# lalitkrajendran/photon

Measured on AMD Instinct MI355X. Metric: Mrays/sec, 1e7-ray 256^3 BOS render, higher is better.
Workload: dtype f32

## Files before the change

### photon_amd/csrc/device_volume_coop.hpp

```cpp
#pragma once
#include "../../include/photon_philox.h"
#include "device_volume.hpp"

namespace photon {

enum PathSlot : int {
    PS_C_COHERENT,
    PS_C_HIT_CELL,
    PS_C_CELL_IN_TILE,
    PS_C_FETCH_UP,
    PS_C_FETCH_DOWN,
    PS_C_TILE_CLAMPED,
    PS_C_INCOHERENT,
    PS_C_INCOHERENT_LANES,
    PS_C_BRICK_PASS,
    PS_C_BRICK_FETCH,
    PS_C_BRICK_REUSED,
    PS_C_BRICK_CLAMPED,
    PS_C_BRICK_LANES,
    PS_C_GATHER_LANES,
    PS_C_SPIN_OUTSIDE,
    PS_C_SPIN_LOW,
    PS_C_SPIN_CAP,
    PS_L_COHERENT,
    PS_L_HIT_A,
    PS_L_HIT_B,
    PS_L_TILE_B_LANES,
    PS_L_FETCH,
    PS_L_FETCH_TWO,
    PS_L_FETCH_TO_B,
    PS_L_FETCH_DOWN,
    PS_L_BASE_AHEAD,
    PS_L_BASE_BEHIND,
    PS_L_TILE_CLAMPED,
    PS_L_NO_FREE_TILE,
    PS_L_OUT_OF_REACH,
    PS_L_MARK_INCOHERENT,
    PS_L_TILES_SKIPPED,
    PS_L_RETRY,
    PS_L_COHERENT_AGAIN,
    PS_L_INCOHERENT,
    PS_L_INCOHERENT_LANES,
    PS_L_BRICK_PASS,
    PS_L_BRICK_FETCH,
    PS_L_BRICK_REUSED,
    PS_L_BRICK_CLAMPED,
    PS_L_BRICK_LANES,
    PS_L_GATHER_LANES,
    PS_L_SPIN_OUTSIDE,
    PS_L_SPIN_CAP,
    PS_L_LOW,
    PS_L_REPAIR_LANES,
    PS_L_KEEP_PREV_LANES,
    PS_COUNT
};
constexpr int kPathSlots = PS_COUNT;
#ifndef PHOTON_PATH_STATS
#define PHOTON_PATH_STATS 0
#endif
#if PHOTON_PATH_STATS
__device__ unsigned long long g_path_stats[kPathSlots];
__device__ __forceinline__ void path_stat(PathSlot k, unsigned long long n = 1) {
    if ((int)(threadIdx.x & 63) == __ffsll((long long)ballot(true)) - 1) atomicAdd(&g_path_stats[k], n);
}
__device__ __forceinline__ void path_stat_if(PathSlot k, bool c) { if (c) path_stat(k); }
__device__ __forceinline__ void path_lanes(PathSlot k, unsigned long long mask) { if (mask != 0) path_stat(k, (unsigned long long)__popcll(mask)); }
#else
#define path_stat(...) ((void)0)
#define path_stat_if(...) ((void)0)
#define path_lanes(...) ((void)0)
#endif

#ifndef PHOTON_BRICK_PASSES
#define PHOTON_BRICK_PASSES 6
#endif
#ifndef PHOTON_LINEAR_TILE_LAYERS
#define PHOTON_LINEAR_TILE_LAYERS 16
#endif
#ifndef PHOTON_LINEAR_TILES
#define PHOTON_LINEAR_TILES 2
#endif
#ifndef PHOTON_TILE_RETRY_MASK
#define PHOTON_TILE_RETRY_MASK 15
#endif
#ifndef PHOTON_BRICK_PITCH
#define PHOTON_BRICK_PITCH 12
#endif
constexpr int kBrickPitch = PHOTON_BRICK_PITCH;
constexpr int kBrickSlab = 8 * kBrickPitch;
#ifndef PHOTON_CUBIC_TILE_LAYERS
#define PHOTON_CUBIC_TILE_LAYERS 7
#endif
constexpr int kCubicTileLayers = PHOTON_CUBIC_TILE_LAYERS;
static_assert(kCubicTileLayers >= 4 && kCubicTileLayers <= 8, "PHOTON_CUBIC_TILE_LAYERS");
template <int INTERP> constexpr int tile_texels() { return INTERP == 2 ? 16 * kCubicTileLayers : PHOTON_LINEAR_TILES * PHOTON_LINEAR_TILE_LAYERS * 4; }
#ifndef PHOTON_SPINS_IN_LDS
#define PHOTON_SPINS_IN_LDS 1
#endif
constexpr int kSpinSlotTexels = PHOTON_SPINS_IN_LDS ? 32 : 0;
template <int INTERP> constexpr int wave_lds_texels() { return tile_texels<INTERP>() + (INTERP == 2 ? 4 : 2) * kBrickSlab + (INTERP == 1 ? kSpinSlotTexels : 0); }
constexpr int kWaveLdsTexels = wave_lds_texels<2>();

template <int RS, int SS>
__device__ __forceinline__ f4 cubic_taps_lds(const f4 *blk, const float (&wx)[4], const float (&wy)[4],
                                             const float (&wz)[4]) {
    float wxy[4][4];
#pragma unroll
    for (int b = 0; b < 4; b++)
#pragma unroll
        for (int a = 0; a < 4; a++) wxy[b][a] = wx[a] * wy[b];
    f4 acc = f4{0, 0, 0, 0}, s = f4{0, 0, 0, 0};
    float w0 = wxy[0][0];
    f4 t[4];
#pragma unroll
    for (int a = 0; a < 4; a++) t[a] = ldtexel(blk + a);
#pragma unroll
    for (int r = 0; r < 16; r++) {
        const int b = r & 3, c = r >> 2;
#pragma unroll
        for (int a = 0; a < 4; a++) {
            const f4 ta = t[a];
            const float w = (a == 0 && b == 0) ? w0 : wxy[b][a];
            if (a == 0 && b == 0) s = f4{w * ta.x, w * ta.y, w * ta.z, w * ta.w};
            else s = f4{fmaf(w, ta.x, s.x), fmaf(w, ta.y, s.y), fmaf(w, ta.z, s.z), fmaf(w, ta.w, s.w)};
            asm volatile("" : "+v"(s.x), "+v"(s.y), "+v"(s.z), "+v"(s.w) : : "memory");
            if (r < 15) t[a] = ldtexel(blk + ((r + 1) >> 2) * SS + ((r + 1) & 3) * RS + a);
            asm volatile("" : "+v"(w0) : : "memory");
        }
        if (b == 3) {
            if (c == 0) acc = f4{wz[0] * s.x, wz[0] * s.y, wz[0] * s.z, wz[0] * s.w};
            else acc = f4{fmaf(wz[c], s.x, acc.x), fmaf(wz[c], s.y, acc.y), fmaf(wz[c], s.z, acc.z), fmaf(wz[c], s.w, acc.w)};
            asm volatile("" : "+v"(acc.x), "+v"(acc.y), "+v"(acc.z), "+v"(acc.w) : : "memory");
        }
    }
    return acc;
}

#define PH_DPP_ROW0 \
    "v_mul_f32_dpp %0, %8, %12 row_newbcast:0 row_mask:0xf bank_mask:0xf\n\t" \
    "v_mul_f32_dpp %1, %9, %12 row_newbcast:0 row_mask:0xf bank_mask:0xf\n\t" \
    "v_mul_f32_dpp %2, %10, %12 row_newbcast:0 row_mask:0xf bank_mask:0xf\n\t" \
    "v_mul_f32_dpp %3, %11, %12 row_newbcast:0 row_mask:0xf bank_mask:0xf\n\t" \
    "v_fmac_f32_dpp %0, %8, %13 row_newbcast:1 row_mask:0xf bank_mask:0xf\n\t" \
    "v_fmac_f32_dpp %1, %9, %13 row_newbcast:1 row_mask:0xf bank_mask:0xf\n\t" \
    "v_fmac_f32_dpp %2, %10, %13 row_newbcast:1 row_mask:0xf bank_mask:0xf\n\t" \
    "v_fmac_f32_dpp %3, %11, %13 row_newbcast:1 row_mask:0xf bank_mask:0xf\n\t" \
    "v_fmac_f32_dpp %0, %8, %14 row_newbcast:2 row_mask:0xf bank_mask:0xf\n\t" \
    "v_fmac_f32_dpp %1, %9, %14 row_newbcast:2 row_mask:0xf bank_mask:0xf\n\t" \
    "v_fmac_f32_dpp %2, %10, %14 row_newbcast:2 row_mask:0xf bank_mask:0xf\n\t" \
    "v_fmac_f32_dpp %3, %11, %14 row_newbcast:2 row_mask:0xf bank_mask:0xf\n\t" \
    "v_fmac_f32_dpp %0, %8, %15 row_newbcast:3 row_mask:0xf bank_mask:0xf\n\t" \
    "v_fmac_f32_dpp %1, %9, %15 row_newbcast:3 row_mask:0xf bank_mask:0xf\n\t" \
    "v_fmac_f32_dpp %2, %10, %15 row_newbcast:3 row_mask:0xf bank_mask:0xf\n\t" \
    "v_fmac_f32_dpp %3, %11, %15 row_newbcast:3 row_mask:0xf bank_mask:0xf\n\t"
#define PH_DPP_ROW1 \
    "v_fmac_f32_dpp %0, %8, %16 row_newbcast:4 row_mask:0xf bank_mask:0xf\n\t" \
    "v_fmac_f32_dpp %1, %9, %16 row_newbcast:4 row_mask:0xf bank_mask:0xf\n\t" \
    "v_fmac_f32_dpp %2, %10, %16 row_newbcast:4 row_mask:0xf bank_mask:0xf\n\t" \
    "v_fmac_f32_dpp %3, %11, %16 row_newbcast:4 row_mask:0xf bank_mask:0xf\n\t" \
    "v_fmac_f32_dpp %0, %8, %17 row_newbcast:5 row_mask:0xf bank_mask:0xf\n\t" \
    "v_fmac_f32_dpp %1, %9, %17 row_newbcast:5 row_mask:0xf bank_mask:0xf\n\t" \
    "v_fmac_f32_dpp %2, %10, %17 row_newbcast:5 row_mask:0xf bank_mask:0xf\n\t" \
    "v_fmac_f32_dpp %3, %11, %17 row_newbcast:5 row_mask:0xf bank_mask:0xf\n\t" \
    "v_fmac_f32_dpp %0, %8, %18 row_newbcast:6 row_mask:0xf bank_mask:0xf\n\t" \
    "v_fmac_f32_dpp %1, %9, %18 row_newbcast:6 row_mask:0xf bank_mask:0xf\n\t" \
    "v_fmac_f32_dpp %2, %10, %18 row_newbcast:6 row_mask:0xf bank_mask:0xf\n\t" \
    "v_fmac_f32_dpp %3, %11, %18 row_newbcast:6 row_mask:0xf bank_mask:0xf\n\t" \
    "v_fmac_f32_dpp %0, %8, %19 row_newbcast:7 row_mask:0xf bank_mask:0xf\n\t" \
    "v_fmac_f32_dpp %1, %9, %19 row_newbcast:7 row_mask:0xf bank_mask:0xf\n\t" \
    "v_fmac_f32_dpp %2, %10, %19 row_newbcast:7 row_mask:0xf bank_mask:0xf\n\t" \
    "v_fmac_f32_dpp %3, %11, %19 row_newbcast:7 row_mask:0xf bank_mask:0xf\n\t"
#define PH_DPP_ROW2 \
    "v_fmac_f32_dpp %0, %8, %20 row_newbcast:8 row_mask:0xf bank_mask:0xf\n\t" \
    "v_fmac_f32_dpp %1, %9, %20 row_newbcast:8 row_mask:0xf bank_mask:0xf\n\t" \
    "v_fmac_f32_dpp %2, %10, %20 row_newbcast:8 row_mask:0xf bank_mask:0xf\n\t" \
    "v_fmac_f32_dpp %3, %11, %20 row_newbcast:8 row_mask:0xf bank_mask:0xf\n\t" \
    "v_fmac_f32_dpp %0, %8, %21 row_newbcast:9 row_mask:0xf bank_mask:0xf\n\t" \
    "v_fmac_f32_dpp %1, %9, %21 row_newbcast:9 row_mask:0xf bank_mask:0xf\n\t" \
    "v_fmac_f32_dpp %2, %10, %21 row_newbcast:9 row_mask:0xf bank_mask:0xf\n\t" \
    "v_fmac_f32_dpp %3, %11, %21 row_newbcast:9 row_mask:0xf bank_mask:0xf\n\t" \
    "v_fmac_f32_dpp %0, %8, %22 row_newbcast:10 row_mask:0xf bank_mask:0xf\n\t" \
    "v_fmac_f32_dpp %1, %9, %22 row_newbcast:10 row_mask:0xf bank_mask:0xf\n\t" \
    "v_fmac_f32_dpp %2, %10, %22 row_newbcast:10 row_mask:0xf bank_mask:0xf\n\t" \
    "v_fmac_f32_dpp %3, %11, %22 row_newbcast:10 row_mask:0xf bank_mask:0xf\n\t" \
    "v_fmac_f32_dpp %0, %8, %23 row_newbcast:11 row_mask:0xf bank_mask:0xf\n\t" \
    "v_fmac_f32_dpp %1, %9, %23 row_newbcast:11 row_mask:0xf bank_mask:0xf\n\t" \
    "v_fmac_f32_dpp %2, %10, %23 row_newbcast:11 row_mask:0xf bank_mask:0xf\n\t" \
    "v_fmac_f32_dpp %3, %11, %23 row_newbcast:11 row_mask:0xf bank_mask:0xf\n\t"
#define PH_DPP_ROW3 \
    "v_fmac_f32_dpp %0, %8, %24 row_newbcast:12 row_mask:0xf bank_mask:0xf\n\t" \
    "v_fmac_f32_dpp %1, %9, %24 row_newbcast:12 row_mask:0xf bank_mask:0xf\n\t" \
    "v_fmac_f32_dpp %2, %10, %24 row_newbcast:12 row_mask:0xf bank_mask:0xf\n\t" \
    "v_fmac_f32_dpp %3, %11, %24 row_newbcast:12 row_mask:0xf bank_mask:0xf\n\t" \
    "v_fmac_f32_dpp %0, %8, %25 row_newbcast:13 row_mask:0xf bank_mask:0xf\n\t" \
    "v_fmac_f32_dpp %1, %9, %25 row_newbcast:13 row_mask:0xf bank_mask:0xf\n\t" \
    "v_fmac_f32_dpp %2, %10, %25 row_newbcast:13 row_mask:0xf bank_mask:0xf\n\t" \
    "v_fmac_f32_dpp %3, %11, %25 row_newbcast:13 row_mask:0xf bank_mask:0xf\n\t" \
    "v_fmac_f32_dpp %0, %8, %26 row_newbcast:14 row_mask:0xf bank_mask:0xf\n\t" \
    "v_fmac_f32_dpp %1, %9, %26 row_newbcast:14 row_mask:0xf bank_mask:0xf\n\t" \
    "v_fmac_f32_dpp %2, %10, %26 row_newbcast:14 row_mask:0xf bank_mask:0xf\n\t" \
    "v_fmac_f32_dpp %3, %11, %26 row_newbcast:14 row_mask:0xf bank_mask:0xf\n\t" \
    "v_fmac_f32_dpp %0, %8, %27 row_newbcast:15 row_mask:0xf bank_mask:0xf\n\t" \
    "v_fmac_f32_dpp %1, %9, %27 row_newbcast:15 row_mask:0xf bank_mask:0xf\n\t" \
    "v_fmac_f32_dpp %2, %10, %27 row_newbcast:15 row_mask:0xf bank_mask:0xf\n\t" \
    "v_fmac_f32_dpp %3, %11, %27 row_newbcast:15 row_mask:0xf bank_mask:0xf\n\t"
#define PH_DPP_ROWS_TEXT PH_DPP_ROW0 PH_DPP_ROW1 PH_DPP_ROW2 PH_DPP_ROW3
#define PH_DS_OFF1 "16"
#define PH_DS_OFF2 "32"
#define PH_DS_OFF3 "48"
#ifndef PHOTON_PRIO_BASE
#define PHOTON_PRIO_BASE 1
#endif
#ifndef PHOTON_PRIO_BLEND
#define PHOTON_PRIO_BLEND 0
#endif
#ifndef PHOTON_PRIO_TAPS_DPP
#define PHOTON_PRIO_TAPS_DPP 3
#endif
#ifndef PHOTON_PRIO_TAPS_LDS
#define PHOTON_PRIO_TAPS_LDS 0
#endif
#ifndef PHOTON_PRIO_BRICK
#define PHOTON_PRIO_BRICK 2
#endif
#ifndef PHOTON_DPP_SLABS
#define PHOTON_DPP_SLABS 3
#endif
constexpr int kDppSlabs = PHOTON_DPP_SLABS;
static_assert(kDppSlabs >= 1 && kDppSlabs <= 4, "PHOTON_DPP_SLABS");
#define PH_DPP_OPERANDS(S, T) \
            : "=&v"(S.x), "=&v"(S.y), "=&v"(S.z), "=&v"(S.w), "=&v"(d0), "=&v"(d1), "=&v"(d2), "=&v"(d3) \
            : "v"(T.x), "v"(T.y), "v"(T.z), "v"(T.w), "v"(wxy[0][0]), "v"(wxy[0][1]), "v"(wxy[0][2]), "v"(wxy[0][3]), \
              "v"(wxy[1][0]), "v"(wxy[1][1]), "v"(wxy[1][2]), "v"(wxy[1][3]), "v"(wxy[2][0]), "v"(wxy[2][1]), "v"(wxy[2][2]), \
              "v"(wxy[2][3]), "v"(wxy[3][0]), "v"(wxy[3][1]), "v"(wxy[3][2]), "v"(wxy[3][3]) \
            : "memory"
__device__ __forceinline__ void dpp_slab(f4 &s, const f4 &tex, const float (&wxy)[4][4]) {
    float d0, d1, d2, d3;
    asm volatile("s_nop 4\n\t" PH_DPP_ROWS_TEXT PH_DPP_OPERANDS(s, tex));
}
__device__ __forceinline__ f4 cubic_taps_hybrid(const f4 *blk, const f4 &reg, const f4 (&more)[3], const float (&wx)[4], const float (&wy)[4],
                                                const float (&wz)[4]) {
    typedef float v4f __attribute__((ext_vector_type(4)));
    constexpr int R = 4 * kDppSlabs;
    float wxy[4][4];
#pragma unroll
    for (int b = 0; b < 4; b++)
#pragma unroll
        for (int a = 0; a < 4; a++) wxy[b][a] = wx[a] * wy[b];
    v4f t0, t1, t2, t3;
    f4 s;
    const unsigned lds = (unsigned)(size_t)blk + 64u * R;
#if PHOTON_PRIO_TAPS_DPP != PHOTON_PRIO_BASE
    __builtin_amdgcn_s_setprio(PHOTON_PRIO_TAPS_DPP);
#endif
    if (R < 16)
    asm volatile(
            "ds_read_b128 %4, %28\n\t"
            "ds_read_b128 %5, %28 offset:" PH_DS_OFF1 "\n\t"
            "ds_read_b128 %6, %28 offset:" PH_DS_OFF2 "\n\t"
            "ds_read_b128 %7, %28 offset:" PH_DS_OFF3 "\n\t"
            "s_nop 4\n\t"
            PH_DPP_ROWS_TEXT
            "s_waitcnt lgkmcnt(0)"
            : "=&v"(s.x), "=&v"(s.y), "=&v"(s.z), "=&v"(s.w), "=&v"(t0), "=&v"(t1), "=&v"(t2), "=&v"(t3)
            : "v"(reg.x), "v"(reg.y), "v"(reg.z), "v"(reg.w), "v"(wxy[0][0]), "v"(wxy[0][1]), "v"(wxy[0][2]), "v"(wxy[0][3]),
              "v"(wxy[1][0]), "v"(wxy[1][1]), "v"(wxy[1][2]), "v"(wxy[1][3]), "v"(wxy[2][0]), "v"(wxy[2][1]), "v"(wxy[2][2]),
              "v"(wxy[2][3]), "v"(wxy[3][0]), "v"(wxy[3][1]), "v"(wxy[3][2]), "v"(wxy[3][3]), "v"(lds)
            : "memory");
    else {
        dpp_slab(s, reg, wxy);
        t0 = t1 = t2 = t3 = v4f{0, 0, 0, 0};
    }
    f4 acc = f4{wz[0] * s.x, wz[0] * s.y, wz[0] * s.z, wz[0] * s.w};
#pragma unroll
    for (int z = 1; z < kDppSlabs; z++) {
        dpp_slab(s, more[z - 1], wxy);
        acc = f4{fmaf(wz[z], s.x, acc.x), fmaf(wz[z], s.y, acc.y), fmaf(wz[z], s.z, acc.z), fmaf(wz[z], s.w, acc.w)};
        asm volatile("" : "+v"(acc.x), "+v"(acc.y), "+v"(acc.z), "+v"(acc.w) : : "memory");
    }
#if PHOTON_PRIO_TAPS_DPP != PHOTON_PRIO_TAPS_LDS
    __builtin_amdgcn_s_setprio(PHOTON_PRIO_TAPS_LDS);
#endif
    f4 t[4] = {f4{t0.x, t0.y, t0.z, t0.w}, f4{t1.x, t1.y, t1.z, t1.w}, f4{t2.x, t2.y, t2.z, t2.w}, f4{t3.x, t3.y, t3.z, t3.w}};
    float w0 = wxy[0][0];
#pragma unroll
    for (int r = R; r < 16; r++) {
        const int b = r & 3, c = r >> 2;
#pragma unroll
        for (int a = 0; a < 4; a++) {
            const f4 ta = t[a];
            const float w = (a == 0 && b == 0) ? w0 : wxy[b][a];
            if (a == 0 && b == 0) s = f4{w * ta.x, w * ta.y, w * ta.z, w * ta.w};
            else s = f4{fmaf(w, ta.x, s.x), fmaf(w, ta.y, s.y), fmaf(w, ta.z, s.z), fmaf(w, ta.w, s.w)};
            asm volatile("" : "+v"(s.x), "+v"(s.y), "+v"(s.z), "+v"(s.w) : : "memory");
            if (r < 15) t[a] = ldtexel(blk + ((r + 1) >> 2) * 16 + ((r + 1) & 3) * 4 + a);
            asm volatile("" : "+v"(w0) : : "memory");
        }
        if (b == 3) {
            if (c == 0) acc = f4{wz[0] * s.x, wz[0] * s.y, wz[0] * s.z, wz[0] * s.w};
            else acc = f4{fmaf(wz[c], s.x, acc.x), fmaf(wz[c], s.y, acc.y), fmaf(wz[c], s.z, acc.z), fmaf(wz[c], s.w, acc.w)};
            asm volatile("" : "+v"(acc.x), "+v"(acc.y), "+v"(acc.z), "+v"(acc.w) : : "memory");
        }
    }
#if PHOTON_PRIO_TAPS_LDS != PHOTON_PRIO_BASE
    __builtin_amdgcn_s_setprio(PHOTON_PRIO_BASE);
#endif
    return acc;
}

__device__ __forceinline__ bool lane_of(unsigned long long mask) { return __builtin_amdgcn_inverse_ballot_w64(mask); }

struct Parked { int ti, tj, tk; int bi, bj, bk; f4 reg; int ci, cj, k0, coff; int ui, uj, uk; f4 more[3]; };
__device__ __forceinline__ Parked parked_none() {
    return Parked{0x7fffffff, 0x7fffffff, 0x7fffffff, 0x7fffffff, 0x7fffffff, 0x7fffffff, f4{0, 0, 0, 0}, 0x7fffffff, 0x7fffffff, 0, 0, 0x7fffffff, 0x7fffffff, 0x7fffffff, {f4{0, 0, 0, 0}, f4{0, 0, 0, 0}, f4{0, 0, 0, 0}}};
}

struct Lead { int i, j, k; };
__device__ __forceinline__ Lead lead_of(unsigned long long todo, float fi, float fj, float fk) {
    const int leader = __ffsll((long long)todo) - 1;
    return Lead{__builtin_amdgcn_readlane(__float_as_int(fi), leader), __builtin_amdgcn_readlane(__float_as_int(fj), leader),
                __builtin_amdgcn_readlane(__float_as_int(fk), leader)};
}
__device__ __forceinline__ unsigned long long same_block(const Lead &c, float fi, float fj, float fk) {
    return ballot(__float_as_int(fi) == c.i) & ballot(__float_as_int(fj) == c.j) & ballot(__float_as_int(fk) == c.k);
}

__device__ __forceinline__ f4 tex3d_cubic_coop(const VolumeDev &v, const f4 *__restrict__ tex, f4 *blk, unsigned long long need,
                                               float x, float y, float z, Parked &parked) {
    f4 *const brick = blk + tile_texels<2>();
    const float xg = x - 0.5f, yg = y - 0.5f, zg = z - 0.5f;
    const float fi = floorf(xg), fj = floorf(yg), fk = floorf(zg);
    float wx[4], wy[4], wz[4];
    bspline_weights(xg - fi, wx[0], wx[1], wx[2], wx[3]);
    bspline_weights(yg - fj, wy[0], wy[1], wy[2], wy[3]);
    bspline_weights(zg - fk, wz[0], wz[1], wz[2], wz[3]);
    const int lane = threadIdx.x & 63;
    if (need == 0) return f4{0, 0, 0, 0};
    {
        constexpr int TL = kCubicTileLayers;
        bool hit = false;
        if (parked.ti != 0x7fffffff) {
            asm volatile("");
            hit = ((ballot(__float_as_int(fi) == parked.ti) & ballot(__float_as_int(fj) == parked.tj) & ballot(__float_as_int(fk) == parked.tk)) & need) == need;
            path_stat_if(PS_C_HIT_CELL, hit);
        }
        if (!hit) {
            const Lead c = lead_of(need, fi, fj, fk);
            if ((same_block(c, fi, fj, fk) & need) == need) {
                const int ck = (int)__int_as_float(c.k);
                int dz = ck - parked.k0;
                if (c.i != parked.ci || c.j != parked.cj || (unsigned)dz > (unsigned)(TL - 4)) {
                    const int ci = (int)__int_as_float(c.i), cj = (int)__int_as_float(c.j);
                    const bool down = c.i == parked.ci && c.j == parked.cj && dz < 0;
                    const int k0 = down ? ck - (TL - 4) : ck;
                    path_stat(down ? PS_C_FETCH_DOWN : PS_C_FETCH_UP);
                    path_stat_if(PS_C_TILE_CLAMPED, ci < 1 || ci + 2 > v.nx - 1 || cj < 1 || cj + 2 > v.ny - 1 || k0 < 1 || k0 + TL - 2 > v.nz - 1);
                    __builtin_amdgcn_wave_barrier();
                    int l = lane;
                    asm volatile("" : "+v"(l));
                    const int tx = clampi(ci - 1 + (l & 3), 0, v.nx - 1), ty = clampi(cj - 1 + ((l >> 2) & 3), 0, v.ny - 1);
#pragma unroll
                    for (int j = 0; j < (TL + 3) / 4; j++) {
                        if (TL % 4 == 0 || j < TL / 4 || l < 16 * (TL % 4)) {
                            const int tz = clampi(k0 - 1 + (l >> 4) + 4 * j, 0, v.nz - 1);
                            const f4 t = ldtexel(tex + (unsigned)((tz * v.ny + ty) * v.nx + tx));
                            *reinterpret_cast<float4 *>(blk + l + 64 * j) = make_float4(t.x, t.y, t.z, t.w);
                        }
                    }
                    __builtin_amdgcn_wave_barrier();
                    parked.ci = c.i; parked.cj = c.j; parked.k0 = k0;
                    dz = ck - k0;
                } else {
                    path_stat(PS_C_CELL_IN_TILE);
                }
                parked.coff = dz * 16;
                parked.reg = ldtexel(blk + parked.coff + (lane & 15));
#pragma unroll
                for (int z = 1; z < kDppSlabs; z++) parked.more[z - 1] = ldtexel(blk + parked.coff + 16 * z + (lane & 15));
                parked.ti = c.i; parked.tj = c.j; parked.tk = c.k;
                hit = true;
            }
        }
        if (hit) {
            path_stat(PS_C_COHERENT);
            const f4 *cell = blk + parked.coff;
            const f4 acc = cubic_taps_hybrid(cell, parked.reg, parked.more, wx, wy, wz);
            __builtin_amdgcn_wave_barrier();
            return acc;
        }
        parked.ti = 0x7fffffff;
    }
    const int bi = (int)fi, bj = (int)fj, bk = (int)fk;
    f4 acc = f4{0, 0, 0, 0};
    bool done = !lane_of(need);
    unsigned long long todo = need;
    path_stat(PS_C_INCOHERENT);
    path_lanes(PS_C_INCOHERENT_LANES, need);
#pragma unroll 1
    for (int pass = 0; pass < PHOTON_BRICK_PASSES && todo != 0; pass++) {
        const int leader = __ffsll((long long)todo) - 1;
        const int ci = __builtin_amdgcn_readlane(bi, leader), cj = __builtin_amdgcn_readlane(bj, leader),
                  ck = __builtin_amdgcn_readlane(bk, leader);
        const int di = bi - ci + 2, dj = bj - cj + 2;
        const bool in_brick = !done && bk == ck && (unsigned)di <= 4u && (unsigned)dj <= 4u;
        path_stat(PS_C_BRICK_PASS);
        path_lanes(PS_C_BRICK_LANES, ballot(in_brick));
        path_stat(ci != parked.bi || cj != parked.bj || ck != parked.bk ? PS_C_BRICK_FETCH : PS_C_BRICK_REUSED);
        if (ci != parked.bi || cj != parked.bj || ck != parked.bk) {
            path_stat_if(PS_C_BRICK_CLAMPED, ci < 3 || ci + 4 > v.nx - 1 || cj < 3 || cj + 4 > v.ny - 1 || ck < 1 || ck + 2 > v.nz - 1);
            __builtin_amdgcn_wave_barrier();
            int l = lane;
            asm volatile("" : "+v"(l));
            const int slot = (l & 7) + ((l >> 3) & 7) * kBrickPitch;
#pragma unroll
            for (int j = 0; j < 4; j++) {
                const int t = l + 64 * j;
                const int tx = clampi(ci - 3 + (t & 7), 0, v.nx - 1), ty = clampi(cj - 3 + ((t >> 3) & 7), 0, v.ny - 1),
                          tz = clampi(ck - 1 + (t >> 6), 0, v.nz - 1);
                const f4 tv = ldtexel(tex + (unsigned)((tz * v.ny + ty) * v.nx + tx));
                *reinterpret_cast<float4 *>(brick + slot + j * kBrickSlab) = make_float4(tv.x, tv.y, tv.z, tv.w);
            }
            __builtin_amdgcn_wave_barrier();
            parked.bi = ci; parked.bj = cj; parked.bk = ck;
        }
        if (in_brick) {
#if PHOTON_PRIO_BRICK != PHOTON_PRIO_BASE
            __builtin_amdgcn_s_setprio(PHOTON_PRIO_BRICK);
#endif
            acc = cubic_taps_lds<kBrickPitch, kBrickSlab>(brick + (dj * kBrickPitch + di), wx, wy, wz);
#if PHOTON_PRIO_BRICK != PHOTON_PRIO_BASE
            __builtin_amdgcn_s_setprio(PHOTON_PRIO_BASE);
#endif
            done = true;
        }
        __builtin_amdgcn_wave_barrier();
        todo = ballot(!done);
    }
    path_lanes(PS_C_GATHER_LANES, ballot(!done));
    if (!done) acc = cubic_gather_fn(tex, v.nx, v.ny, v.nz, x, y, z);
    return acc;
}

__device__ __attribute__((noinline)) f4 linear_gather_fn(const f4 *__restrict__ tex, int nx, int ny, int nz, float x,
                                                         float y, float z, float weight_scale, float weight_inv) {
    const float xb = x - 0.5f, yb = y - 0.5f, zb = z - 0.5f;
    const float fi = floorf(xb), fj = floorf(yb), fk = floorf(zb);
    const float a = quant_weight(xb - fi, weight_scale, weight_inv), b = quant_weight(yb - fj, weight_scale, weight_inv),
                c = quant_weight(zb - fk, weight_scale, weight_inv);
    const int i = (int)fi, j = (int)fj, k = (int)fk;
    const int i0 = clampi(i, 0, nx - 1), i1 = clampi(i + 1, 0, nx - 1);
    const int j0 = clampi(j, 0, ny - 1), j1 = clampi(j + 1, 0, ny - 1);
    const int k0 = clampi(k, 0, nz - 1), k1 = clampi(k + 1, 0, nz - 1);
    auto row = [&](int kk, int jj) {
        const f4 *r = tex + (unsigned)((kk * ny + jj) * nx);
        f4 v = lerp4(ldtexel(r + i0), ldtexel(r + i1), a);
        asm volatile("" : "+v"(v.x), "+v"(v.y), "+v"(v.z), "+v"(v.w));
        return v;
    };
    const f4 c00 = row(k0, j0), c10 = row(k0, j1);
    f4 c0 = lerp4(c00, c10, b);
    asm volatile("" : "+v"(c0.x), "+v"(c0.y), "+v"(c0.z), "+v"(c0.w));
    const f4 c01 = row(k1, j0), c11 = row(k1, j1);
    const f4 c1 = lerp4(c01, c11, b);
    return lerp4(c0, c1, c);
}

__device__ __forceinline__ float uniformf(float x) {
    float s;
    asm("s_nop 0\n\tv_readfirstlane_b32 %0, %1\n\ts_nop 4" : "=s"(s) : "v"(x));
    return s;
}

__device__ __forceinline__ float pair_swap(float v) {
    return __int_as_float(__builtin_amdgcn_update_dpp(0, __float_as_int(v), 0xB1 , 0xF, 0xF, false));
}

template <bool QUANT, bool PIN = false>
__device__ __forceinline__ f4 tex3d_linear_coop(const VolumeDev &v, const f4 *__restrict__ tex, f4 *blk, unsigned long long need,
                                                float x, float y, float z, Parked &parked, unsigned tick = 0) {
    f4 *const brick = blk + tile_texels<1>();
    const float xb = x - 0.5f, yb = y - 0.5f, zb = z - 0.5f;
    const float fi = floorf(xb), fj = floorf(yb), fk = floorf(zb);
    float a = xb - fi, b = yb - fj, c = zb - fk;
    if (QUANT) {
        a = floorf(fmaf(a, v.weight_scale, 0.5f)) * v.weight_inv;

        b = floorf(fmaf(b, v.weight_scale, 0.5f)) * v.weight_inv;
        c = floorf(fmaf(c, v.weight_scale, 0.5f)) * v.weight_inv;
    }
    const int lane = threadIdx.x & 63;
    if (need == 0) return f4{0, 0, 0, 0};
    {
        constexpr int TL = PHOTON_LINEAR_TILE_LAYERS;
        constexpr int NT = PHOTON_LINEAR_TILES;
        static_assert(TL == 4 || TL == 8 || TL == 16, "PHOTON_LINEAR_TILE_LAYERS");
        static_assert(NT == 1 || NT == 2, "PHOTON_LINEAR_TILES");
        constexpr unsigned kDzMax = (unsigned)(TL - 2);
        constexpr int kIncoherent = 0x7ffffffe;
        const int fib = __float_as_int(fi), fjb = __float_as_int(fj);
        unsigned dzq = 0;
        unsigned long long ok_a = 0, ok_b = 0;
        bool hit = false;
        if (parked.ti != 0x7fffffff) {
            asm volatile("");
            dzq = (unsigned)(int)(fk - __int_as_float(parked.tk));
            ok_a = ballot(fib == parked.ti) & ballot(fjb == parked.tj) & ballot(dzq <= kDzMax);
            hit = (ok_a & need) == need;
            path_stat_if(PS_L_HIT_A, hit);
            if (NT == 2 && !hit && parked.ui < kIncoherent) {
                const unsigned dzu = (unsigned)(int)(fk - __int_as_float(parked.uk));
                ok_b = ballot(fib == parked.ui) & ballot(fjb == parked.uj) & ballot(dzu <= kDzMax);
                if (((ok_a | ok_b) & need) == need) {
                    hit = true;
                    path_stat(PS_L_HIT_B);
                    dzq = lane_of(ok_a) ? dzq : dzu + TL;
                }
            }
        }
        path_stat_if(PS_L_TILES_SKIPPED, !hit && parked.ui == kIncoherent && (tick & (unsigned)PHOTON_TILE_RETRY_MASK) != 0);
        path_stat_if(PS_L_RETRY, !hit && parked.ui == kIncoherent && (tick & (unsigned)PHOTON_TILE_RETRY_MASK) == 0);
        if (!hit && (parked.ui != kIncoherent || (tick & (unsigned)PHOTON_TILE_RETRY_MASK) == 0)) {
            const unsigned long long rest = need & ~(ok_a | ok_b);
            const Lead l1 = lead_of(rest, fi, fj, fk);
            const unsigned long long col1 = rest & ballot(fib == l1.i) & ballot(fjb == l1.j), rest2 = rest & ~col1;
            Lead l2 = l1;
            unsigned long long col2 = 0;
            int n_new = 1;
            if (rest2 != 0) {
                l2 = lead_of(rest2, fi, fj, fk);
                col2 = rest2 & ballot(fib == l2.i) & ballot(fjb == l2.j);
                n_new = (rest2 & ~col2) != 0 ? 3 : 2;
            }
            const bool free_a = (ok_a & need) == 0, free_b = NT == 2 && (ok_b & need) == 0;
            path_stat_if(PS_L_NO_FREE_TILE, n_new > (free_a ? 1 : 0) + (free_b ? 1 : 0));
            if (n_new <= (free_a ? 1 : 0) + (free_b ? 1 : 0)) {
                path_stat_if(PS_L_FETCH_TWO, n_new == 2);
#pragma unroll 1
                for (int j = 0; j < n_new; j++) {
                    path_stat(PS_L_FETCH);
                    const bool to_a = j == 0 && free_a;
                    const Lead ld = j == 0 ? l1 : l2;
                    const unsigned long long lanes = j == 0 ? col1 : col2;
                    const int oi = to_a ? parked.ti : parked.ui, oj = to_a ? parked.tj : parked.uj, ok = to_a ? parked.tk : parked.uk;
                    const float klf = __int_as_float(ld.k);
                    const bool behind = (lanes & ballot(fk < klf)) != 0, ahead = (lanes & ballot(fk > klf)) != 0;
                    const bool down = ld.i == oi && ld.j == oj && klf < __int_as_float(ok);
                    const int ci = (int)__int_as_float(ld.i), cj = (int)__int_as_float(ld.j);
                    const int base = (int)klf - (down ? (ahead ? TL - 3 : TL - 2) : (behind ? 1 : 0));
                    f4 *const tile = blk + (to_a ? 0 : 4 * TL);
                    path_stat_if(PS_L_FETCH_TO_B, !to_a);
                    path_stat_if(PS_L_FETCH_DOWN, down);
                    path_stat_if(PS_L_BASE_AHEAD, down && ahead);
                    path_stat_if(PS_L_BASE_BEHIND, !down && behind);
                    path_stat_if(PS_L_TILE_CLAMPED, ci < 0 || ci + 1 > v.nx - 1 || cj < 0 || cj + 1 > v.ny - 1 || base < 0 || base + TL - 1 > v.nz - 1);
                    __builtin_amdgcn_wave_barrier();
                    if (lane < 4 * TL) {
                        int l = lane;
                        if (PIN) asm volatile("" : "+v"(l));
                        const int tx = clampi(ci + (l & 1), 0, v.nx - 1), ty = clampi(cj + ((l >> 1) & 1), 0, v.ny - 1),
                                  tz = clampi(base + (l >> 2), 0, v.nz - 1);
                        const f4 t = ldtexel(tex + (unsigned)((tz * v.ny + ty) * v.nx + tx));
                        const f4 o = f4{pair_swap(t.x), pair_swap(t.y), pair_swap(t.z), pair_swap(t.w)};
                        const bool hi = (l & 1) != 0;
                        *reinterpret_cast<float4 *>(tile + l) = make_float4(hi ? t.x - o.x : t.x, hi ? t.y - o.y : t.y,
                                                                            hi ? t.z - o.z : t.z, hi ? t.w - o.w : t.w);
                    }
                    __builtin_amdgcn_wave_barrier();
                    const int basef = __float_as_int(uniformf((float)base));
                    if (to_a) { parked.ti = ld.i; parked.tj = ld.j; parked.tk = basef; }
                    else { parked.ui = ld.i; parked.uj = ld.j; parked.uk = basef; }
                }
                dzq = (unsigned)(int)(fk - __int_as_float(parked.tk));
                ok_a = ballot(fib == parked.ti) & ballot(fjb == parked.tj) & ballot(dzq <= kDzMax);
                if (NT == 2 && parked.ui < kIncoherent) {
                    const unsigned dzu = (unsigned)(int)(fk - __int_as_float(parked.uk));
                    ok_b = ballot(fib == parked.ui) & ballot(fjb == parked.uj) & ballot(dzu <= kDzMax);
                    dzq = lane_of(ok_a) ? dzq : dzu + TL;
                }
                hit = ((ok_a | ok_b) & need) == need;
                path_stat_if(PS_L_OUT_OF_REACH, !hit);
                path_stat_if(PS_L_COHERENT_AGAIN, hit && parked.ui == kIncoherent);
                if (hit && parked.ui == kIncoherent) parked.ui = 0x7fffffff;
            }
        }
        if (hit) {
            path_stat(PS_L_COHERENT);
            path_lanes(PS_L_TILE_B_LANES, need & ~ok_a);
            const f4 *q = blk + ((dzq & (unsigned)(NT * TL - 1)) << 2);
#if PHOTON_PRIO_BLEND != PHOTON_PRIO_BASE
            __builtin_amdgcn_s_setprio(PHOTON_PRIO_BLEND);
#endif
            const f4 c00 = lerp4d(ldtexel(q), ldtexel(q + 1), a), c10 = lerp4d(ldtexel(q + 2), ldtexel(q + 3), a);
            const f4 c01 = lerp4d(ldtexel(q + 4), ldtexel(q + 5), a), c11 = lerp4d(ldtexel(q + 6), ldtexel(q + 7), a);
            const f4 c0 = lerp4(c00, c10, b), c1 = lerp4(c01, c11, b);
            const f4 acc = lerp4(c0, c1, c);
#if PHOTON_PRIO_BLEND != PHOTON_PRIO_BASE
            __builtin_amdgcn_s_setprio(PHOTON_PRIO_BASE);
#endif
            __builtin_amdgcn_wave_barrier();
            return acc;
        }
        path_stat_if(PS_L_MARK_INCOHERENT, parked.ui != kIncoherent);
        parked.ti = 0x7fffffff;
        parked.ui = kIncoherent;
    }
    const int bi = (int)fi, bj = (int)fj, bk = (int)fk;
    f4 acc = f4{0, 0, 0, 0};
    bool done = !lane_of(need);
    unsigned long long todo = need;
    path_stat(PS_L_INCOHERENT);
    path_lanes(PS_L_INCOHERENT_LANES, need);
#pragma unroll 1
    for (int pass = 0; pass < PHOTON_BRICK_PASSES && todo != 0; pass++) {
        const int leader = __ffsll((long long)todo) - 1;
        const int ci = __builtin_amdgcn_readlane(bi, leader), cj = __builtin_amdgcn_readlane(bj, leader),
                  ck = __builtin_amdgcn_readlane(bk, leader);
        const int di = bi - ci + 3, dj = bj - cj + 3;
        const bool in_brick = !done && bk == ck && (unsigned)di <= 6u && (unsigned)dj <= 6u;
        path_stat(PS_L_BRICK_PASS);
        path_lanes(PS_L_BRICK_LANES, ballot(in_brick));
        path_stat(ci != parked.bi || cj != parked.bj || ck != parked.bk ? PS_L_BRICK_FETCH : PS_L_BRICK_REUSED);
        if (ci != parked.bi || cj != parked.bj || ck != parked.bk) {
            path_stat_if(PS_L_BRICK_CLAMPED, ci < 3 || ci + 4 > v.nx - 1 || cj < 3 || cj + 4 > v.ny - 1 || ck < 0 || ck + 1 > v.nz - 1);
            __builtin_amdgcn_wave_barrier();
            int l = lane;
            asm volatile("" : "+v"(l));
            const int slot = (l & 7) + ((l >> 3) & 7) * kBrickPitch;
#pragma unroll
            for (int j = 0; j < 2; j++) {
                const int t = l + 64 * j;
                const int tx = clampi(ci - 3 + (t & 7), 0, v.nx - 1), ty = clampi(cj - 3 + ((t >> 3) & 7), 0, v.ny - 1),
                          tz = clampi(ck + (t >> 6), 0, v.nz - 1);
                const f4 tv = ldtexel(tex + (unsigned)((tz * v.ny + ty) * v.nx + tx));
                *reinterpret_cast<float4 *>(brick + slot + j * kBrickSlab) = make_float4(tv.x, tv.y, tv.z, tv.w);
            }
            __builtin_amdgcn_wave_barrier();
            parked.bi = ci; parked.bj = cj; parked.bk = ck;
        }
        if (in_brick) {
#if PHOTON_PRIO_BLEND != PHOTON_PRIO_BASE
            __builtin_amdgcn_s_setprio(PHOTON_PRIO_BLEND);
#endif
            const f4 *q = brick + (dj * kBrickPitch + di);
            const f4 c00 = lerp4(ldtexel(q), ldtexel(q + 1), a), c10 = lerp4(ldtexel(q + kBrickPitch), ldtexel(q + kBrickPitch + 1), a);
            const f4 c01 = lerp4(ldtexel(q + kBrickSlab), ldtexel(q + kBrickSlab + 1), a),
                     c11 = lerp4(ldtexel(q + kBrickSlab + kBrickPitch), ldtexel(q + kBrickSlab + kBrickPitch + 1), a);
            const f4 c0 = lerp4(c00, c10, b), c1 = lerp4(c01, c11, b);
            acc = lerp4(c0, c1, c);
#if PHOTON_PRIO_BLEND != PHOTON_PRIO_BASE
            __builtin_amdgcn_s_setprio(PHOTON_PRIO_BASE);
#endif
            done = true;
        }
        __builtin_amdgcn_wave_barrier();
        todo = ballot(!done);
    }
    path_lanes(PS_L_GATHER_LANES, ballot(!done));
    if (!done) acc = linear_gather_fn(tex, v.nx, v.ny, v.nz, x, y, z, v.weight_scale, v.weight_inv);
    return acc;
}

struct MarchU {
    float minx, miny, minz, maxx, maxy, maxz;
    float sx, sy, sz;
    float nxm2, nym2, nzm2;
    float fnx, fny, fnz;
    float step, data_min, spin_step;
    int nx, ny, nz;
};
__device__ __forceinline__ MarchU make_march_consts(const VolumeDev &v, f3 scale) {
    MarchU u;
    u.minx = uniformf(v.min_bound.x); u.miny = uniformf(v.min_bound.y); u.minz = uniformf(v.min_bound.z);
    u.maxx = uniformf(v.max_bound.x); u.maxy = uniformf(v.max_bound.y); u.maxz = uniformf(v.max_bound.z);
    u.sx = uniformf(scale.x); u.sy = uniformf(scale.y); u.sz = uniformf(scale.z);
    u.nxm2 = uniformf((float)(v.nx - 2)); u.nym2 = uniformf((float)(v.ny - 2)); u.nzm2 = uniformf((float)(v.nz - 2));
    u.fnx = uniformf((float)v.nx); u.fny = uniformf((float)v.ny); u.fnz = uniformf((float)v.nz);
    u.step = uniformf(v.step_size); u.data_min = uniformf(v.data_min);
    u.spin_step = uniformf(v.step_size / (1 + v.data_min));
    u.nx = v.nx; u.ny = v.ny; u.nz = v.nz;
    return u;
}
__device__ __forceinline__ f3 lookup_index_u(f3 pos, const MarchU &u) {
    const f3 off = mk3(pos.x - u.minx, pos.y - u.miny, pos.z - u.minz);
    const f3 fn = mk3(u.sx * off.x, u.sy * off.y, u.sz * off.z);
    return mk3(1 + fn.x * u.nxm2, 1 + fn.y * u.nym2, 1 + fn.z * u.nzm2);
}
__device__ __forceinline__ unsigned long long access_mask(const MarchU &u, f3 l) {
    return ~(ballot(l.x < 0) | ballot(l.y < 0) | ballot(l.z < 0) | ballot(l.x >= u.fnx) | ballot(l.y >= u.fny) | ballot(l.z >= u.fnz));
}
__device__ __forceinline__ unsigned long long inside_mask(f3 p, const MarchU &u) {
    return ~(ballot(p.x < u.minx) | ballot(p.y < u.miny) | ballot(p.z < u.minz) | ballot(p.x >= u.maxx) | ballot(p.y >= u.maxy) | ballot(p.z >= u.maxz));
}

struct WaveCount { unsigned iterations; unsigned samples; };
__device__ __forceinline__ void count_samples(MarchCount &mc, unsigned long long m) { if (lane_of(m)) mc.samples++; }
__device__ __forceinline__ void count_iterations(MarchCount &mc, unsigned long long m) { if (lane_of(m)) mc.iterations++; }
__device__ __forceinline__ void count_samples(WaveCount &mc, unsigned long long m) { mc.samples += (unsigned)__popcll(m); }
__device__ __forceinline__ void count_iterations(WaveCount &mc, unsigned long long m) { mc.iterations += (unsigned)__popcll(m); }

struct PrevVal {
    f4 v;
    __device__ __forceinline__ void init(f4 *, f4 x) { v = x; }
    __device__ __forceinline__ void set(f4 x) { v = x; }
    __device__ __forceinline__ f4 get() const { return v; }
};

template <int INTERP, bool QUANT, class CNT, bool PIN = false>
__device__ __forceinline__ f4 sample_coop(const VolumeDev &v, const f4 *__restrict__ tex, f4 *blk, unsigned long long need, f3 lookup,
                                          const PrevVal &prev, float data_min, CNT &mc, Parked &parked, unsigned tick = 0) {
    f4 val = INTERP == 1 ? tex3d_linear_coop<QUANT, PIN>(v, tex, blk, need, lookup.x, lookup.y, lookup.z, parked, tick)
                         : tex3d_cubic_coop(v, tex, blk, need, lookup.x, lookup.y, lookup.z, parked);
    count_samples(mc, need);
    if (INTERP == 1) {
        const unsigned long long low = need & ballot(val.w < data_min);
        if (low != 0) {
            const float ambient = 1.000277;
            const f4 val_prev = prev.get();
            const unsigned long long repair = low & ballot(val_prev.w == 0);
            path_stat(PS_L_LOW);
            path_lanes(PS_L_REPAIR_LANES, repair);
            path_lanes(PS_L_KEEP_PREV_LANES, low & ~repair);
            if (repair != 0) {
                count_samples(mc, repair);
                if (lane_of(repair)) {
                    const f4 t = linear_gather_fn(tex, v.nx, v.ny, v.nz, lookup.x, lookup.y, lookup.z - 1, v.weight_scale, v.weight_inv);
                    val = f4{t.x, t.y, t.z, ambient - 1};
                }
            }
            if (lane_of(low & ~repair)) val = val_prev;
        }
    }
    return val;
}

struct MarchResume {
    int loop_ctr, spins;
    f4 val_prev;
    unsigned max_trips;
    unsigned trips_base;
    bool fresh;
};
__device__ __forceinline__ MarchResume resume_fresh() { return MarchResume{0, 0, f4{0, 0, 0, 0}, ~0u, 0u, true}; }

template <int INTERP, bool SAVE, bool QUANT, class CNT>
__device__ __forceinline__ unsigned long long rk4_coop(bool active_lane, f3 &rpos, f3 &rdir, const VolumeDev &v,
                                                       const f4 *__restrict__ tex, f4 *blk, f3 scale, CNT &mc,
                                                       const InterDump &idump, MarchResume &rs) {
    const MarchU u = make_march_consts(v, scale);
    int loop_ctr = rs.loop_ctr;
    constexpr bool kSpinLds = PHOTON_SPINS_IN_LDS && INTERP == 1;
    int spins = rs.spins;
    int *const spin_slot = reinterpret_cast<int *>(blk + tile_texels<1>() + 2 * kBrickSlab) + (threadIdx.x & 63);
    if (kSpinLds) *spin_slot = spins;
    int *const ctr_slot = spin_slot + 64;
    if (kSpinLds) *ctr_slot = loop_ctr;
    unsigned trips = rs.trips_base;
    const unsigned trips_end = rs.max_trips == ~0u ? ~0u : trips + rs.max_trips;
    Parked parked = parked_none();
    PrevVal prev{};
    if (INTERP == 1) prev.init(blk, rs.val_prev);
    unsigned long long active = ballot(active_lane);
    unsigned long long first = active & ballot(loop_ctr == 0);
    while (active != 0 && trips < trips_end) {
        f3 lookup = lookup_index_u(rpos, u);
        const unsigned long long in_a = inside_mask(rpos, u);
        unsigned long long not_over = ~0ull;
        if (trips > (unsigned)kLoopMax) not_over = ~ballot((kSpinLds ? *ctr_slot : loop_ctr) > kLoopMax);
        trips++;
        if (SAVE && INTERP == 1) { if (lane_of(active & not_over)) record_intermediate(idump, kSpinLds ? *ctr_slot : loop_ctr, rpos, rdir); }
        const unsigned long long alive = active & not_over & (in_a | first);
        unsigned long long go = alive, spin = 0;
        if ((alive & ~in_a) != 0) {
            const unsigned long long access = access_mask(u, lookup);
// ... 162 lines not shown
```

### photon_amd/path_stats.py

```python
from __future__ import annotations

import ctypes
import os
import re

HEADER = os.path.join(os.path.dirname(os.path.abspath(__file__)), "csrc", "device_volume_coop.hpp")

SLOTS = (
    "C_COHERENT", "C_HIT_CELL", "C_CELL_IN_TILE", "C_FETCH_UP", "C_FETCH_DOWN", "C_TILE_CLAMPED",
    "C_INCOHERENT", "C_INCOHERENT_LANES", "C_BRICK_PASS", "C_BRICK_FETCH", "C_BRICK_REUSED", "C_BRICK_CLAMPED",
    "C_BRICK_LANES", "C_GATHER_LANES", "C_SPIN_OUTSIDE", "C_SPIN_LOW", "C_SPIN_CAP",
    "L_COHERENT", "L_HIT_A", "L_HIT_B", "L_TILE_B_LANES", "L_FETCH", "L_FETCH_TWO", "L_FETCH_TO_B", "L_FETCH_DOWN",
    "L_BASE_AHEAD", "L_BASE_BEHIND", "L_TILE_CLAMPED", "L_NO_FREE_TILE", "L_OUT_OF_REACH", "L_MARK_INCOHERENT",
    "L_TILES_SKIPPED", "L_RETRY", "L_COHERENT_AGAIN", "L_INCOHERENT", "L_INCOHERENT_LANES", "L_BRICK_PASS",
    "L_BRICK_FETCH", "L_BRICK_REUSED", "L_BRICK_CLAMPED", "L_BRICK_LANES", "L_GATHER_LANES", "L_SPIN_OUTSIDE",
    "L_SPIN_CAP", "L_LOW", "L_REPAIR_LANES", "L_KEEP_PREV_LANES",
)

OPTICS_HEADER = os.path.join(os.path.dirname(os.path.abspath(__file__)), "csrc", "device_optics.hpp")

SPLAT_SLOTS = (
    "E_WAVES", "E_COOP", "E_FALLBACK", "E_FB_WIDE", "E_FB_TILES", "E_FB_RADIUS",
    "E_SHARED_X_LANES", "E_BOTH_X_LANES", "E_SHARED_Y_LANES", "E_BOTH_Y_LANES", "E_CLIPPED_LANES", "E_LANE_CLIPPED_LANES",
    "E_TILES", "E_TILES_SAME", "E_TILES_MIXED", "E_MULTI_TILE",
    "T_WAVES", "T_COOP", "T_LANE_ROUTE", "T_MULTI_TILE", "T_TAPS_LANDED", "T_TAPS_DROPPED", "T_TAPS_WRAPPED",
    "K_GEN_ERF", "K_STATE_ERF", "K_GEN_TRAIN", "K_STATE_TRAIN", "K_GEN_TAPS", "K_STATE_TAPS",
)

PATH_STATS_FLAGS = ("-DPHOTON_PATH_STATS=1",)


def header_slots(path: str = HEADER):
    with open(path) as f:
        text = f.read()
    body = re.search(r"enum PathSlot\s*:\s*int\s*\{(.*?)\};", text, re.S).group(1)
    names = re.findall(r"^\s*PS_(\w+)\s*,", body, re.M)
    assert names and names[-1] != "COUNT"
    return tuple(names)


def header_splat_slots(path: str = OPTICS_HEADER):
    with open(path) as f:
        text = f.read()
    body = re.search(r"enum SplatSlot\s*:\s*int\s*\{(.*?)\};", text, re.S).group(1)
    names = re.findall(r"^\s*SS_(\w+)\s*,", body, re.M)
    assert names and names[-1] != "COUNT"
    return tuple(names)


def read_splat(lib) -> dict:
    f = lib.lib.photon_debug_splat_stats
    f.argtypes = [ctypes.c_void_p, ctypes.c_int]
    f.restype = ctypes.c_int
    out = (ctypes.c_ulonglong * len(SPLAT_SLOTS))()
    rc = f(ctypes.cast(out, ctypes.c_void_p), len(SPLAT_SLOTS))
    if rc != 0:
        raise RuntimeError(f"photon_debug_splat_stats failed ({rc})")
    return dict(zip(SPLAT_SLOTS, (int(v) for v in out)))


def read(lib) -> dict:
    f = lib.lib.photon_debug_path_stats
    f.argtypes = [ctypes.c_void_p, ctypes.c_int]
    f.restype = ctypes.c_int
    out = (ctypes.c_ulonglong * len(SLOTS))()
    rc = f(ctypes.cast(out, ctypes.c_void_p), len(SLOTS))
    if rc != 0:
        raise RuntimeError(f"photon_debug_path_stats failed ({rc})")
    return dict(zip(SLOTS, (int(v) for v in out)))
```

Baseline: 188.8.

## Test parked-cell hits by fractional offset and advance along z without leader

Replaces the per-sample floor plus three-ballot cell-identity check with an unsigned-bit range test on the offset from a parked cell origin, computed with a single max3 and one ballot. When only the z cell changes by one, the wave advances the parked cell up or down directly, with no leader readlane and no same-block ballots. B-spline weights are now computed from those offsets only after the path is chosen. This shortens the common coherent path for rays marching through the volume, at the cost of extra parked state and a second ballot sequence when the first test misses.

```diff
diff --git a/photon_amd/csrc/device_volume_coop.hpp b/photon_amd/csrc/device_volume_coop.hpp
--- a/photon_amd/csrc/device_volume_coop.hpp
+++ b/photon_amd/csrc/device_volume_coop.hpp
@@ -52,6 +52,7 @@
     PS_L_LOW,
     PS_L_REPAIR_LANES,
     PS_L_KEEP_PREV_LANES,
+    PS_C_ADVANCE_NO_LEAD,
     PS_COUNT
 };
 constexpr int kPathSlots = PS_COUNT;
@@ -310,9 +311,23 @@
 
 __device__ __forceinline__ bool lane_of(unsigned long long mask) { return __builtin_amdgcn_inverse_ballot_w64(mask); }
 
-struct Parked { int ti, tj, tk; int bi, bj, bk; f4 reg; int ci, cj, k0, coff; int ui, uj, uk; f4 more[3]; };
+struct Parked { int ti, tj, tk; int bi, bj, bk; f4 reg; int ci, cj, k0, coff; int ui, uj, uk; f4 more[3]; float cx, cy, cz; };
 __device__ __forceinline__ Parked parked_none() {
-    return Parked{0x7fffffff, 0x7fffffff, 0x7fffffff, 0x7fffffff, 0x7fffffff, 0x7fffffff, f4{0, 0, 0, 0}, 0x7fffffff, 0x7fffffff, 0, 0, 0x7fffffff, 0x7fffffff, 0x7fffffff, {f4{0, 0, 0, 0}, f4{0, 0, 0, 0}, f4{0, 0, 0, 0}}};
+    return Parked{0x7fffffff, 0x7fffffff, 0x7fffffff, 0x7fffffff, 0x7fffffff, 0x7fffffff, f4{0, 0, 0, 0}, 0x7fffffff, 0x7fffffff, 0, 0, 0x7fffffff, 0x7fffffff, 0x7fffffff, {f4{0, 0, 0, 0}, f4{0, 0, 0, 0}, f4{0, 0, 0, 0}},
+                  __int_as_float(0x7fffffff), 0.0f, 0.0f};
+}
+
+constexpr unsigned kOneBits = 0x3f800000u;
+__device__ __forceinline__ unsigned umax3(unsigned a, unsigned b, unsigned c) {
+    unsigned m;
+    asm("v_max3_u32 %0, %1, %2, %3" : "=v"(m) : "v"(a), "v"(b), "v"(c));
+    return m;
+}
+
+__device__ __forceinline__ float uniformf(float x) {
+    float s;
+    asm("s_nop 0\n\tv_readfirstlane_b32 %0, %1\n\ts_nop 4" : "=s"(s) : "v"(x));
+    return s;
 }
 
 struct Lead { int i, j, k; };
@@ -328,68 +343,100 @@
 __device__ __forceinline__ f4 tex3d_cubic_coop(const VolumeDev &v, const f4 *__restrict__ tex, f4 *blk, unsigned long long need,
                                                float x, float y, float z, Parked &parked) {
     f4 *const brick = blk + tile_texels<2>();
-    const float xg = x - 0.5f, yg = y - 0.5f, zg = z - 0.5f;
-    const float fi = floorf(xg), fj = floorf(yg), fk = floorf(zg);
-    float wx[4], wy[4], wz[4];
-    bspline_weights(xg - fi, wx[0], wx[1], wx[2], wx[3]);
-    bspline_weights(yg - fj, wy[0], wy[1], wy[2], wy[3]);
-    bspline_weights(zg - fk, wz[0], wz[1], wz[2], wz[3]);
     const int lane = threadIdx.x & 63;
     if (need == 0) return f4{0, 0, 0, 0};
+    float ax, ay, az;
+    float fi, fj, fk;
+    bool hit = false;
+    float wx[4], wy[4], wz[4];
     {
         constexpr int TL = kCubicTileLayers;
-        bool hit = false;
-        if (parked.ti != 0x7fffffff) {
-            asm volatile("");
-            hit = ((ballot(__float_as_int(fi) == parked.ti) & ballot(__float_as_int(fj) == parked.tj) & ballot(__float_as_int(fk) == parked.tk)) & need) == need;
+        auto enter_cell = [&](bool same_column, int ck) {
+            int dz = ck - parked.k0;
+            if (!same_column || (unsigned)dz > (unsigned)(TL - 4)) {
+                const int ci = (int)__int_as_float(parked.ci), cj = (int)__int_as_float(parked.cj);
+                const bool down = same_column && dz < 0;
+                const int k0 = down ? ck - (TL - 4) : ck;
+                path_stat(down ? PS_C_FETCH_DOWN : PS_C_FETCH_UP);
+                path_stat_if(PS_C_TILE_CLAMPED, ci < 1 || ci + 2 > v.nx - 1 || cj < 1 || cj + 2 > v.ny - 1 || k0 < 1 || k0 + TL - 2 > v.nz - 1);
+                __builtin_amdgcn_wave_barrier();
+                int l = lane;
+                asm volatile("" : "+v"(l));
+                const int tx = clampi(ci - 1 + (l & 3), 0, v.nx - 1), ty = clampi(cj - 1 + ((l >> 2) & 3), 0, v.ny - 1);
+#pragma unroll
+                for (int j = 0; j < (TL + 3) / 4; j++) {
+                    if (TL % 4 == 0 || j < TL / 4 || l < 16 * (TL % 4)) {
+                        const int tz = clampi(k0 - 1 + (l >> 4) + 4 * j, 0, v.nz - 1);
+                        const f4 t = ldtexel(tex + (unsigned)((tz * v.ny + ty) * v.nx + tx));
+                        *reinterpret_cast<float4 *>(blk + l + 64 * j) = make_float4(t.x, t.y, t.z, t.w);
+                    }
+                }
+                __builtin_amdgcn_wave_barrier();
+                parked.k0 = k0;
+                dz = ck - k0;
+            } else {
+                path_stat(PS_C_CELL_IN_TILE);
+            }
+            parked.coff = dz * 16;
+            parked.reg = ldtexel(blk + parked.coff + (lane & 15));
+#pragma unroll
+            for (int z = 1; z < kDppSlabs; z++) parked.more[z - 1] = ldtexel(blk + parked.coff + 16 * z + (lane & 15));
+        };
+        if (__float_as_int(parked.cx) != 0x7fffffff) {
+            ax = x - parked.cx; ay = y - parked.cy; az = z - parked.cz;
+            const unsigned bx = (unsigned)__float_as_int(ax), by = (unsigned)__float_as_int(ay);
+            hit = (ballot(umax3(bx, by, (unsigned)__float_as_int(az)) < kOneBits) & need) == need;
             path_stat_if(PS_C_HIT_CELL, hit);
+            if (!hit && (ballot((bx > by ? bx : by) < kOneBits) & need) == need) {
+                const int ck = parked.k0 + (parked.coff >> 4);
+                float cz = parked.cz - 1.0f;
+                int ck_to = ck - 1;
+                az = z - cz;
+                hit = ck >= 1 && (ballot((unsigned)__float_as_int(az) < kOneBits) & need) == need;
+                if (!hit) {
+                    cz = parked.cz + 1.0f;
+                    ck_to = ck + 1;
+                    az = z - cz;
+                    hit = (ballot((unsigned)__float_as_int(az) < kOneBits) & need) == need;
+                }
+                if (hit) {
+                    path_stat(PS_C_ADVANCE_NO_LEAD);
+                    parked.cz = uniformf(cz);
+                    enter_cell(true, ck_to);
+                }
+            }
         }
         if (!hit) {
+            const float xg = x - 0.5f, yg = y - 0.5f, zg = z - 0.5f;
+            fi = floorf(xg); fj = floorf(yg); fk = floorf(zg);
+            ax = xg - fi; ay = yg - fj; az = zg - fk;
             const Lead c = lead_of(need, fi, fj, fk);
             if ((same_block(c, fi, fj, fk) & need) == need) {
-                const int ck = (int)__int_as_float(c.k);
-                int dz = ck - parked.k0;
-                if (c.i != parked.ci || c.j != parked.cj || (unsigned)dz > (unsigned)(TL - 4)) {
-                    const int ci = (int)__int_as_float(c.i), cj = (int)__int_as_float(c.j);
-                    const bool down = c.i == parked.ci && c.j == parked.cj && dz < 0;
-                    const int k0 = down ? ck - (TL - 4) : ck;
-                    path_stat(down ? PS_C_FETCH_DOWN : PS_C_FETCH_UP);
-                    path_stat_if(PS_C_TILE_CLAMPED, ci < 1 || ci + 2 > v.nx - 1 || cj < 1 || cj + 2 > v.ny - 1 || k0 < 1 || k0 + TL - 2 > v.nz - 1);
-                    __builtin_amdgcn_wave_barrier();
-                    int l = lane;
-                    asm volatile("" : "+v"(l));
-                    const int tx = clampi(ci - 1 + (l & 3), 0, v.nx - 1), ty = clampi(cj - 1 + ((l >> 2) & 3), 0, v.ny - 1);
-#pragma unroll
-                    for (int j = 0; j < (TL + 3) / 4; j++) {
-                        if (TL % 4 == 0 || j < TL / 4 || l < 16 * (TL % 4)) {
-                            const int tz = clampi(k0 - 1 + (l >> 4) + 4 * j, 0, v.nz - 1);
-                            const f4 t = ldtexel(tex + (unsigned)((tz * v.ny + ty) * v.nx + tx));
-                            *reinterpret_cast<float4 *>(blk + l + 64 * j) = make_float4(t.x, t.y, t.z, t.w);
-                        }
-                    }
-                    __builtin_amdgcn_wave_barrier();
-                    parked.ci = c.i; parked.cj = c.j; parked.k0 = k0;
-                    dz = ck - k0;
-                } else {
-                    path_stat(PS_C_CELL_IN_TILE);
-                }
-                parked.coff = dz * 16;
-                parked.reg = ldtexel(blk + parked.coff + (lane & 15));
-#pragma unroll
-                for (int z = 1; z < kDppSlabs; z++) parked.more[z - 1] = ldtexel(blk + parked.coff + 16 * z + (lane & 15));
-                parked.ti = c.i; parked.tj = c.j; parked.tk = c.k;
+                parked.cx = (c.i | c.j | c.k) < 0 ? __int_as_float(0x7fffffff) : uniformf(__int_as_float(c.i) + 0.5f);
+                parked.cy = uniformf(__int_as_float(c.j) + 0.5f);
+                parked.cz = uniformf(__int_as_float(c.k) + 0.5f);
+                const bool same_column = c.i == parked.ci && c.j == parked.cj;
+                parked.ci = c.i; parked.cj = c.j;
+                enter_cell(same_column, (int)__int_as_float(c.k));
                 hit = true;
             }
         }
-        if (hit) {
-            path_stat(PS_C_COHERENT);
-            const f4 *cell = blk + parked.coff;
-            const f4 acc = cubic_taps_hybrid(cell, parked.reg, parked.more, wx, wy, wz);
-            __builtin_amdgcn_wave_barrier();
-            return acc;
-        }
-        parked.ti = 0x7fffffff;
-    }
+    }
+    if (__builtin_expect(hit, 1)) {
+        bspline_weights(ax, wx[0], wx[1], wx[2], wx[3]);
+        bspline_weights(ay, wy[0], wy[1], wy[2], wy[3]);
+        bspline_weights(az, wz[0], wz[1], wz[2], wz[3]);
+        path_stat(PS_C_COHERENT);
+        const f4 *cell = blk + parked.coff;
+        const f4 acc = cubic_taps_hybrid(cell, parked.reg, parked.more, wx, wy, wz);
+        __builtin_amdgcn_wave_barrier();
+        return acc;
+    }
+    parked.cx = __int_as_float(0x7fffffff);
+    asm volatile("" : "+v"(ax), "+v"(ay), "+v"(az));
+    bspline_weights(ax, wx[0], wx[1], wx[2], wx[3]);
+    bspline_weights(ay, wy[0], wy[1], wy[2], wy[3]);
+    bspline_weights(az, wz[0], wz[1], wz[2], wz[3]);
     const int bi = (int)fi, bj = (int)fj, bk = (int)fk;
     f4 acc = f4{0, 0, 0, 0};
     bool done = !lane_of(need);
@@ -463,12 +510,6 @@
     const f4 c01 = row(k1, j0), c11 = row(k1, j1);
     const f4 c1 = lerp4(c01, c11, b);
     return lerp4(c0, c1, c);
-}
-
-__device__ __forceinline__ float uniformf(float x) {
-    float s;
-    asm("s_nop 0\n\tv_readfirstlane_b32 %0, %1\n\ts_nop 4" : "=s"(s) : "v"(x));
-    return s;
 }
 
 __device__ __forceinline__ float pair_swap(float v) {
diff --git a/photon_amd/path_stats.py b/photon_amd/path_stats.py
--- a/photon_amd/path_stats.py
+++ b/photon_amd/path_stats.py
@@ -15,6 +15,7 @@
     "L_TILES_SKIPPED", "L_RETRY", "L_COHERENT_AGAIN", "L_INCOHERENT", "L_INCOHERENT_LANES", "L_BRICK_PASS",
     "L_BRICK_FETCH", "L_BRICK_REUSED", "L_BRICK_CLAMPED", "L_BRICK_LANES", "L_GATHER_LANES", "L_SPIN_OUTSIDE",
     "L_SPIN_CAP", "L_LOW", "L_REPAIR_LANES", "L_KEEP_PREV_LANES",
+    "C_ADVANCE_NO_LEAD",
 )
 
 OPTICS_HEADER = os.path.join(os.path.dirname(os.path.abspath(__file__)), "csrc", "device_optics.hpp")
```

Result: faster. 192.7 (median of 6 runs) (+2.1%).
